# taesungp/swapping-autoencoder-pytorch

Measured on NVIDIA H100. Metric: training images/sec, higher is better.
Workload: dtype tf32

## Files before the change

### include/sae_b200.h

```cpp
#ifndef SAE_B200_H_
#define SAE_B200_H_

#include <stdint.h>

#ifdef __cplusplus
extern "C" {
#endif

#define SAE_OK              0
#define SAE_E_INVALID      -1
#define SAE_E_CUDA         -2
#define SAE_E_UNSUPPORTED  -3

#define SAE_ABI_VERSION 15
int         sae_abi_version(void);
const char* sae_last_error(void);
int64_t     sae_launch_count(void);
int         sae_tcgen05_available(void);

int sae_upfirdn2d(const float* input, const float* kernel, float* out,
                  int64_t major, int in_h, int in_w, int minor,
                  int kernel_h, int kernel_w,
                  int up_x, int up_y, int down_x, int down_y,
                  int pad_x0, int pad_x1, int pad_y0, int pad_y1,
                  int round_tf32, void* stream);

int sae_upfirdn2d_separable(const float* input, const float* taps_y, const float* taps_x, float* out,
                            int64_t major, int in_h, int in_w, int minor, int kernel_h, int kernel_w,
                            int up, int down, int pad_x0, int pad_x1, int pad_y0, int pad_y1, int round_tf32, void* stream);

int sae_fused_bias_act(const float* x, const float* bias, const float* ref, float* out,
                       int64_t size_x, int64_t step_b, int size_b,
                       int act, int grad, float alpha, float scale,
                       const float* noise, const float* noise_weight, int64_t noise_div,
                       int round_tf32, void* stream);

int sae_bias_act_backward(const float* grad_out, const float* out, float* grad_in, float* grad_bias,
// ... 45 lines not shown
} sae_conv_geom;

typedef struct sae_conv_epilogue {
    const float* bias;
    const float* noise;
    const float* noise_weight;
    const float* residual;
    float   alpha;
    float   gain;
    float   res_scale;
    int32_t act;
    int32_t round_tf32;
    uint32_t* act_mask;
} sae_conv_epilogue;

int sae_conv2d_fprop(const float* x, const float* w, float* y, const sae_conv_geom* g,
                     const sae_conv_epilogue* epi, int impl, void* stream);
int sae_conv2d_dgrad(const float* dy, const float* wt, float* dx, const sae_conv_geom* g,
                     const sae_conv_epilogue* epi, int impl, void* stream);
int sae_conv2d_wgrad(const float* dy, const float* x, float* dw, const sae_conv_geom* g,
                     int impl, void* stream);

int sae_conv2d_query_impl(const sae_conv_geom* g, int dir);

int sae_split_tf32(const float* x, float* hi, float* lo, int64_t n, void* stream);
int sae_conv2d_fprop_3xtf32(const float* x, const float* w_hi, const float* w_lo, float* y, const sae_conv_geom* g,
                            const sae_conv_epilogue* epi, int impl, void* stream);
int sae_conv2d_dgrad_3xtf32(const float* dy, const float* wt_hi, const float* wt_lo, float* dx, const sae_conv_geom* g,
                            const sae_conv_epilogue* epi, int impl, void* stream);
int sae_conv2d_wgrad_3xtf32(const float* dy, const float* x, float* dw, const sae_conv_geom* g, int impl, void* stream);

int sae_bucket_pack(const float* const* ptrs, const int64_t* offsets, const int64_t* sizes, int n,
                    float* bucket, int64_t total, void* stream);
int sae_bucket_unpack(float* const* ptrs, const int64_t* offsets, const int64_t* sizes, int n,
                      const float* bucket, int64_t total, float scale, void* stream);

int sae_filter_modulate(const float* w_krsc, const float* s, float* out_nkrsc, float* out_ncrsk, int n, int k, int c, int r,
                        int s_, int round_tf32, void* stream);
int sae_conv2d_query_modulated(const sae_conv_geom* g);
int sae_conv2d_fprop_per_sample(const float* x, const float* w_nkrsc, float* y, const sae_conv_geom* g,
                                const sae_conv_epilogue* epi, void* stream);
int sae_conv2d_dgrad_per_sample(const float* dy, const float* w_ncrsk, float* dx, const sae_conv_geom* g,
                                const sae_conv_epilogue* epi, void* stream);
int sae_conv2d_wgrad_modulated(const float* dy, const float* x, const float* s, const float* w_krsc, float* dw, float* ds,
                               const sae_conv_geom* g, void* stream);
int sae_conv2d_fprop_per_sample_3xtf32(const float* x, const float* w_nkrsc_hi, const float* w_nkrsc_lo, float* y,
// ... 61 lines not shown
```

### swapping_autoencoder_pytorch_b200/_lib.py

```python
import ctypes
import os
import subprocess
import threading

_HERE = os.path.dirname(os.path.abspath(__file__))
LIB_PATH = os.path.join(_HERE, "libsae_b200.so")
CSRC_DIR = os.path.join(_HERE, "csrc")

SAE_ABI_VERSION = 15

c_float_p = ctypes.c_void_p
c_stream = ctypes.c_void_p


class ConvGeom(ctypes.Structure):
    _fields_ = [(n, ctypes.c_int32) for n in
                ("N", "H", "W", "C", "K", "R", "S", "P", "Q", "stride", "pad_t", "pad_l")]

    def key(self):
        return tuple(getattr(self, n) for n, _ in self._fields_)


class ConvEpilogue(ctypes.Structure):
    _fields_ = [("bias", ctypes.c_void_p), ("noise", ctypes.c_void_p), ("noise_weight", ctypes.c_void_p),
                ("residual", ctypes.c_void_p), ("alpha", ctypes.c_float), ("gain", ctypes.c_float),
                ("res_scale", ctypes.c_float), ("act", ctypes.c_int32), ("round_tf32", ctypes.c_int32),
                ("act_mask", ctypes.c_void_p)]


SIGNATURES = {
    "sae_abi_version": (ctypes.c_int, []),
    "sae_last_error": (ctypes.c_char_p, []),
# ... 25 lines not shown
                                             ctypes.c_int64, ctypes.c_int, ctypes.c_int, c_stream]),
    "sae_add_scale": (ctypes.c_int, [c_float_p, c_float_p, c_float_p, ctypes.c_int64, ctypes.c_float, ctypes.c_int,
                                     c_stream]),
    "sae_round_tf32": (ctypes.c_int, [c_float_p, c_float_p, ctypes.c_int64, c_stream]),
    "sae_upsample2x_add_scale": (ctypes.c_int, [c_float_p, c_float_p, c_float_p, ctypes.c_int, ctypes.c_int, ctypes.c_int,
                                                ctypes.c_int, ctypes.c_float, ctypes.c_int, c_stream]),
    "sae_upsample2x_backward": (ctypes.c_int, [c_float_p, c_float_p, ctypes.c_int, ctypes.c_int, ctypes.c_int, ctypes.c_int,
                                               ctypes.c_float, ctypes.c_int, c_stream]),
    "sae_filter_prep": (ctypes.c_int, [c_float_p, c_float_p, c_float_p, ctypes.c_int, ctypes.c_int, ctypes.c_int, ctypes.c_int,
                                       ctypes.c_float, ctypes.c_int, c_stream]),
    "sae_filter_unprep": (ctypes.c_int, [c_float_p, c_float_p, ctypes.c_int, ctypes.c_int, ctypes.c_int, ctypes.c_int,
                                         ctypes.c_float, c_stream]),
    "sae_reflect_pad": (ctypes.c_int, [c_float_p, c_float_p] + [ctypes.c_int] * 8 + [c_stream]),
    "sae_reflect_pad_backward": (ctypes.c_int, [c_float_p, c_float_p] + [ctypes.c_int] * 8 + [c_stream]),
    "sae_pad_channels": (ctypes.c_int, [c_float_p, c_float_p, ctypes.c_int64, ctypes.c_int64, ctypes.c_int, ctypes.c_int,
                                        ctypes.c_int64, ctypes.c_int64, ctypes.c_int64, ctypes.c_int, c_stream]),
    "sae_conv2d_fprop": (ctypes.c_int, [c_float_p, c_float_p, c_float_p, ctypes.POINTER(ConvGeom),
                                        ctypes.POINTER(ConvEpilogue), ctypes.c_int, c_stream]),
    "sae_conv2d_dgrad": (ctypes.c_int, [c_float_p, c_float_p, c_float_p, ctypes.POINTER(ConvGeom),
                                        ctypes.POINTER(ConvEpilogue), ctypes.c_int, c_stream]),
    "sae_conv2d_wgrad": (ctypes.c_int, [c_float_p, c_float_p, c_float_p, ctypes.POINTER(ConvGeom), ctypes.c_int,
                                        c_stream]),
    "sae_conv2d_query_impl": (ctypes.c_int, [ctypes.POINTER(ConvGeom), ctypes.c_int]),
    "sae_split_tf32": (ctypes.c_int, [c_float_p, c_float_p, c_float_p, ctypes.c_int64, c_stream]),
    "sae_conv2d_fprop_3xtf32": (ctypes.c_int, [c_float_p, c_float_p, c_float_p, c_float_p, ctypes.POINTER(ConvGeom),
                                               ctypes.POINTER(ConvEpilogue), ctypes.c_int, c_stream]),
    "sae_conv2d_dgrad_3xtf32": (ctypes.c_int, [c_float_p, c_float_p, c_float_p, c_float_p, ctypes.POINTER(ConvGeom),
                                               ctypes.POINTER(ConvEpilogue), ctypes.c_int, c_stream]),
    "sae_conv2d_wgrad_3xtf32": (ctypes.c_int, [c_float_p, c_float_p, c_float_p, ctypes.POINTER(ConvGeom), ctypes.c_int,
                                               c_stream]),
    "sae_bucket_pack": (ctypes.c_int, [ctypes.c_void_p, ctypes.c_void_p, ctypes.c_void_p, ctypes.c_int, c_float_p,
                                       ctypes.c_int64, c_stream]),
    "sae_bucket_unpack": (ctypes.c_int, [ctypes.c_void_p, ctypes.c_void_p, ctypes.c_void_p, ctypes.c_int, c_float_p,
                                         ctypes.c_int64, ctypes.c_float, c_stream]),
    "sae_filter_modulate": (ctypes.c_int, [c_float_p] * 4 + [ctypes.c_int] * 6 + [c_stream]),
    "sae_conv2d_query_modulated": (ctypes.c_int, [ctypes.POINTER(ConvGeom)]),
    "sae_conv2d_fprop_per_sample": (ctypes.c_int, [c_float_p, c_float_p, c_float_p, ctypes.POINTER(ConvGeom),
                                                   ctypes.POINTER(ConvEpilogue), c_stream]),
    "sae_conv2d_dgrad_per_sample": (ctypes.c_int, [c_float_p, c_float_p, c_float_p, ctypes.POINTER(ConvGeom),
                                                   ctypes.POINTER(ConvEpilogue), c_stream]),
    "sae_conv2d_wgrad_modulated": (ctypes.c_int, [c_float_p] * 6 + [ctypes.POINTER(ConvGeom), c_stream]),
    "sae_conv2d_fprop_per_sample_3xtf32": (ctypes.c_int, [c_float_p, c_float_p, c_float_p, c_float_p, ctypes.POINTER(ConvGeom),
                                                          ctypes.POINTER(ConvEpilogue), c_stream]),
    "sae_conv2d_dgrad_per_sample_3xtf32": (ctypes.c_int, [c_float_p, c_float_p, c_float_p, c_float_p, ctypes.POINTER(ConvGeom),
                                                          ctypes.POINTER(ConvEpilogue), c_stream]),
    "sae_conv2d_wgrad_modulated_3xtf32": (ctypes.c_int, [c_float_p] * 6 + [ctypes.POINTER(ConvGeom), c_stream]),
# ... 68 lines not shown
```

### swapping_autoencoder_pytorch_b200/csrc/api.cu

```cuda
#include "conv_internal.cuh"
#include <mutex>

namespace sae {

thread_local char g_err[512] = "";
std::atomic<int64_t> g_launches{0};

int sm_count() {
    static int n = 0;
    static std::once_flag once;
    std::call_once(once, [] {
        int dev = 0;
        if (cudaGetDevice(&dev) != cudaSuccess) dev = 0;
        cudaDeviceProp prop;
        if (cudaGetDeviceProperties(&prop, dev) == cudaSuccess) n = prop.multiProcessorCount;
        if (n <= 0) n = 132;
    });
    return n;
}

static int validate_geom(const sae_conv_geom* g, const char* who) {
    if (!g) return fail(SAE_E_INVALID, "%s: null geometry", who);
    if (g->N < 0 || g->H <= 0 || g->W <= 0 || g->C <= 0 || g->K <= 0 || g->R <= 0 || g->S <= 0 || g->P <= 0 ||
        g->Q <= 0 || g->stride <= 0)
        return fail(SAE_E_INVALID, "%s: non-positive dimension", who);
    if ((int64_t)(g->P - 1) * g->stride - g->pad_t + g->R - 1 < 0 || (int64_t)(g->Q - 1) * g->stride - g->pad_l + g->S - 1 < 0)
        return fail(SAE_E_INVALID, "%s: inconsistent P/Q", who);
    return SAE_OK;
}

}

using namespace sae;

extern "C" int sae_abi_version(void) { return SAE_ABI_VERSION; }
extern "C" const char* sae_last_error(void) { return g_err; }
extern "C" int64_t sae_launch_count(void) { return g_launches.load(std::memory_order_relaxed); }
extern "C" int sae_tcgen05_available(void) { return tc_available() ? 1 : 0; }

extern "C" int sae_conv2d_query_impl(const sae_conv_geom* g, int dir) {
    if (validate_geom(g, "query_impl") != SAE_OK) return SAE_E_INVALID;
    if (!tc_available()) return 1;
    bool ok = dir == 0 ? tc_fprop_eligible(g) : dir == 1 ? tc_dgrad_eligible(g) : wgrad_wg_eligible(g);
    return ok ? 2 : 1;
}

static int conv2d_fprop(const float* x, const float* w, const float* w_lo, float* y, const sae_conv_geom* g,
                        const sae_conv_epilogue* epi, int impl, void* stream, const char* who,
                        void* ws = nullptr, int64_t* ws_bytes = nullptr) {
    int rc = validate_geom(g, who);
    if (rc) return rc;
    const bool det = ws_bytes != nullptr;
    bool query = false;
    if (g->N == 0) return det ? det_workspace(ws, ws_bytes, 0, who, &query) : SAE_OK;
    if (!x || !w || !y) return fail(SAE_E_INVALID, "%s: null pointer", who);
    cudaStream_t st = (cudaStream_t)stream;
    EpiParams e = make_epi(epi);
    const bool tc_ok = (det || tc_available()) && tc_fprop_eligible(g);
    if (impl == 2 && !tc_ok) return fail(SAE_E_UNSUPPORTED, "%s: shape not eligible for the wgmma kernel", who);
    if (impl != 1 && tc_ok) {
        if (det && ((rc = det_workspace(ws, ws_bytes, 0, who, &query)) || query)) return rc;
        return tc_fprop(x, w, y, g, e, st, w_lo);
    }
    GatherParams p;
    p.N = g->N; p.OH = g->P; p.OW = g->Q; p.IH = g->H; p.IW = g->W; p.Cs = g->C; p.R = g->R; p.S = g->S;
    p.SY = g->stride; p.DY = 1; p.OFFY = -g->pad_t; p.OFFX = -g->pad_l; p.DIV = 1;
    p.Ncol = g->K; p.K = g->R * g->S * g->C; p.M = (int64_t)g->N * g->P * g->Q;
// ... 204 lines not shown
```

### swapping_autoencoder_pytorch_b200/csrc/conv_internal.cuh

```cuda
#pragma once
#include "common.cuh"

namespace sae {

struct GatherParams {
    int N, OH, OW;
    int IH, IW, Cs;
    int R, S;
    int SY, DY, OFFY, OFFX, DIV;
    int Ncol;
    int K;
    int64_t M;
};

struct WgradParams {
    int N, H, W, C;
    int Ko, R, S;
    int P, Q;
    int stride, pad_t, pad_l;
    int Ncol;
    int64_t Mpix;
    int64_t chunk;
    int64_t img_pix;
    const float* mod_s;
// ... 13 lines not shown
    return row_tiles * groups_per_tile * splits_per_image * taps;
}

int conv_gather_dispatch(const float* src, const float* wmat, float* out, const GatherParams& p, const EpiParams& e,
                         cudaStream_t st, const float* wlo = nullptr);
int conv_gather_dispatch_det(const float* src, const float* wmat, float* out, const GatherParams& p, const EpiParams& e,
                             cudaStream_t st, const float* wlo, void* ws, int64_t* ws_bytes, const char* who);
int conv_wgrad(const float* dy, const float* x, float* dw, const sae_conv_geom* g, int impl, cudaStream_t st, bool split = false);
bool wgrad_modulated_eligible(const sae_conv_geom* g);
int conv_wgrad_modulated(const float* dy, const float* x, const float* s, const float* w_krsc, float* dw, float* ds,
                         const sae_conv_geom* g, cudaStream_t st, bool split = false);
int conv_wgrad_det(const float* dy, const float* x, float* dw, const sae_conv_geom* g, int impl, cudaStream_t st, bool split,
                   void* ws, int64_t* ws_bytes, const char* who);
int conv_wgrad_modulated_det(const float* dy, const float* x, const float* s, const float* w_krsc, float* dw, float* ds,
                             const sae_conv_geom* g, cudaStream_t st, bool split, void* ws, int64_t* ws_bytes, const char* who);

bool tc_available();
bool tc_fprop_eligible(const sae_conv_geom* g);
bool tc_dgrad_eligible(const sae_conv_geom* g);
int tc_fprop(const float* x, const float* w, float* y, const sae_conv_geom* g, const EpiParams& e, cudaStream_t st,
             const float* w_lo = nullptr);
int tc_dgrad(const float* dy, const float* wt, float* dx, const sae_conv_geom* g, const EpiParams& e, cudaStream_t st,
             const float* wt_lo = nullptr);
bool wgrad_wg_eligible(const sae_conv_geom* g);
int wgrad_wg_launch(const float* dy, const float* x, float* dw, const WgradParams& p, cudaStream_t st, DetWs* det = nullptr);
int wgrad_split_launch(const float* dy, const float* x, float* dw, const WgradParams& p, unsigned splits, cudaStream_t st,
                       const DetWs* det = nullptr);
bool tc_per_sample_eligible(const sae_conv_geom* g, int dgrad);
int tc_conv_per_sample(const float* src, const float* w, float* out, const sae_conv_geom* g, int dgrad, const EpiParams& e,
                       cudaStream_t st, const float* w_lo = nullptr);

}
```

### swapping_autoencoder_pytorch_b200/csrc/conv_wgmma.cu

```cuda
#include "tc_common.cuh"
#include <mutex>

namespace sae {

EncodeTiledFn g_encode = nullptr;
static bool g_tc_ok = false;

static void tc_init_once() {
    static std::once_flag once;
    std::call_once(once, [] {
        int dev = 0;
        if (cudaGetDevice(&dev) != cudaSuccess) return;
        cudaDeviceProp prop;
        if (cudaGetDeviceProperties(&prop, dev) != cudaSuccess) return;
        if (prop.major != 9) return;
        void* fn = nullptr;
        cudaDriverEntryPointQueryResult qres;
        if (cudaGetDriverEntryPoint("cuTensorMapEncodeTiled", &fn, cudaEnableDefault, &qres) != cudaSuccess) return;
        if (qres != cudaDriverEntryPointSuccess || fn == nullptr) return;
        g_encode = (EncodeTiledFn)fn;
        const char* off = getenv("SAE_DISABLE_TCGEN05");
        g_tc_ok = !(off && off[0] == '1');
    });
}
// ... 2 lines not shown
    tc_init_once();
    return g_tc_ok;
}

constexpr int TC_MAX_TAPS = 16;
constexpr int TC_THREADS = 288;
constexpr int TC_CONSUMERS = 256;
constexpr int TC_BK = 32;
constexpr int TC_A_BYTES = 128 * TC_BK * 4;

struct TcParams {
    int num_cblk;
    int ntaps;
    int stride;
    int tw, th, tn;
    int tiles_w, tiles_h, tiles_n;
    int ON, OH, OW, Ncol;
    int src_c;
    int o_mul, o_offy, o_offx;
    int FH, FW;
    short oy[TC_MAX_TAPS], ox[TC_MAX_TAPS];
    int wk[TC_MAX_TAPS];
    int w_nstride;
    EpiParams epi;
};

__device__ __forceinline__ void tc_epilogue_math(float (&v)[32], const EpiParams& e, int colb, int64_t pixel, int ncol, bool valid, float nz) {
    uint32_t pos = 0;
#pragma unroll
    for (int j = 0; j < 32; ++j) {
        float t = v[j];
        if (e.bias) t += __ldg(e.bias + colb + j);
        t += nz;
        pos |= (t > 0.f ? 1u : 0u) << j;
        if (e.act == 3) t = t > 0.f ? t : t * e.alpha;
        t *= e.gain;
        v[j] = t;
    }
    if (e.act_mask && valid) e.act_mask[(pixel * ncol + colb) >> 5] = pos;
    if (e.residual && valid) {
        const float4* r4 = reinterpret_cast<const float4*>(e.residual + pixel * ncol + colb);
#pragma unroll
        for (int j = 0; j < 8; ++j) {
            float4 r = __ldg(r4 + j);
            v[4 * j + 0] = (v[4 * j + 0] + r.x) * e.res_scale;
            v[4 * j + 1] = (v[4 * j + 1] + r.y) * e.res_scale;
// ... 173 lines not shown
        float nz = 0.f;
        if (p.epi.noise && valid) nz = __ldg(p.epi.noise_weight) * __ldg(p.epi.noise + pixel);
        uint8_t* stg = smem_gen + (size_t)ch * TC_A_BYTES + (size_t)row * 128;
        float v[32];
#pragma unroll
        for (int j = 0; j < 8; ++j) {
            const float4 o = *reinterpret_cast<const float4*>(stg + ((j ^ (row & 7)) << 4));
            v[4 * j] = o.x; v[4 * j + 1] = o.y; v[4 * j + 2] = o.z; v[4 * j + 3] = o.w;
        }
        tc_epilogue_math(v, p.epi, col0 + ch * 32, pixel, p.Ncol, valid, nz);
#pragma unroll
        for (int j = 0; j < 8; ++j)
            *reinterpret_cast<float4*>(stg + ((j ^ (row & 7)) << 4)) = make_float4(v[4 * j], v[4 * j + 1], v[4 * j + 2], v[4 * j + 3]);
    }
    asm volatile("fence.proxy.async.shared::cta;" ::: "memory");
    asm volatile("bar.sync 1, %0;" ::"n"(TC_CONSUMERS) : "memory");
    if (threadIdx.x == 0) {
        for (int ch = 0; ch < NCHUNK; ++ch) tma_store_4d(&map_out, base + (uint32_t)ch * TC_A_BYTES, col0 + ch * 32, q0, p0, n0);
        asm volatile("cp.async.bulk.commit_group;" ::: "memory");
        asm volatile("cp.async.bulk.wait_group.read 0;" ::: "memory");
    }
}

int encode_map(CUtensorMap* m, const void* ptr, int rank, const cuuint64_t* dims, const cuuint64_t* strides_bytes,
               const cuuint32_t* box, const cuuint32_t* estr, CUtensorMapSwizzle swizzle) {
    if (g_encode == nullptr && !tc_available()) return fail(SAE_E_UNSUPPORTED, "cuTensorMapEncodeTiled is not available on this device / driver");
    CUresult r = g_encode(m, CU_TENSOR_MAP_DATA_TYPE_FLOAT32, (cuuint32_t)rank, const_cast<void*>(ptr), dims, strides_bytes, box,
                          estr, CU_TENSOR_MAP_INTERLEAVE_NONE, swizzle, CU_TENSOR_MAP_L2_PROMOTION_L2_256B,
                          CU_TENSOR_MAP_FLOAT_OOB_FILL_NONE);
    if (r != CUDA_SUCCESS) return fail(SAE_E_CUDA, "cuTensorMapEncodeTiled failed with CUresult %d", (int)r);
    return SAE_OK;
}

struct TcProblem {
    const float* src; int SN, SH, SW, SC;
    const float* wmat; int Ncol, Ktot;
    const float* wmat_lo;
    int w_per_sample;
    float* out; int OH, OW;
    int o_mul, o_offy, o_offx, FH, FW;
    int stride, ntaps;
    int oy[TC_MAX_TAPS], ox[TC_MAX_TAPS], wk[TC_MAX_TAPS];
};

static bool tc_shape_ok(int src_c, int ncol, int ntaps, int stride, int ow) {
    if (src_c % 32 != 0 || ncol % 32 != 0) return false;
    if (ntaps < 1 || ntaps > TC_MAX_TAPS) return false;
    if (stride != 1 && stride != 2) return false;
    int tw = pow2_ceil(ow) < 16 ? pow2_ceil(ow) : 16;
    if (tw * stride > 256) return false;
    return true;
}

static void tc_fill_params(const TcProblem& pr, const EpiParams& e, TcParams& p) {
    p.num_cblk = pr.SC / 32;
    p.ntaps = pr.ntaps;
    p.stride = pr.stride;
    tile_box(pr.OH, pr.OW, 128, 16, p.tw, p.th, p.tn);
    p.tiles_w = (pr.OW + p.tw - 1) / p.tw;
    p.tiles_h = (pr.OH + p.th - 1) / p.th;
    p.tiles_n = (pr.SN + p.tn - 1) / p.tn;
    p.ON = pr.SN; p.OH = pr.OH; p.OW = pr.OW; p.Ncol = pr.Ncol; p.src_c = pr.SC;
    for (int t = 0; t < pr.ntaps; ++t) { p.oy[t] = (short)pr.oy[t]; p.ox[t] = (short)pr.ox[t]; p.wk[t] = pr.wk[t]; }
    p.o_mul = pr.o_mul; p.o_offy = pr.o_offy; p.o_offx = pr.o_offx; p.FH = pr.FH; p.FW = pr.FW;
    p.w_nstride = pr.w_per_sample ? pr.Ncol : 0;
    p.epi = e;
}

static int tc_encode_filter(const TcProblem& pr, const float* wmat, int b_rows, CUtensorMap* mw) {
    cuuint64_t dims[2] = {(cuuint64_t)pr.Ktot, (cuuint64_t)pr.Ncol * (cuuint64_t)(pr.w_per_sample ? pr.SN : 1)};
    cuuint64_t strides[1] = {(cuuint64_t)pr.Ktot * 4};
    cuuint32_t box[2] = {32, (cuuint32_t)b_rows};
    cuuint32_t es[2] = {1, 1};
    return encode_map(mw, wmat, 2, dims, strides, box, es);
}

int encode_act_map(CUtensorMap* m, const float* ptr, int N, int H, int W, int C, int tw, int th, int tn, int stride) {
    cuuint64_t dims[4] = {(cuuint64_t)C, (cuuint64_t)W, (cuuint64_t)H, (cuuint64_t)N};
    cuuint64_t strides[3] = {(cuuint64_t)C * 4, (cuuint64_t)W * C * 4, (cuuint64_t)H * W * C * 4};
    cuuint32_t box[4] = {32, (cuuint32_t)(tw * stride), (cuuint32_t)(th * stride), (cuuint32_t)tn};
    cuuint32_t es[4] = {1, (cuuint32_t)stride, (cuuint32_t)stride, 1};
    return encode_map(m, ptr, 4, dims, strides, box, es);
}

static int tc_encode_maps(const TcProblem& pr, const TcParams& p, int b_rows, CUtensorMap* msrc, CUtensorMap* mw, CUtensorMap* mout) {
    {
        int rc = encode_act_map(msrc, pr.src, pr.SN, pr.SH, pr.SW, pr.SC, p.tw, p.th, p.tn, pr.stride);
        if (rc) return rc;
    }
    {
        int rc = tc_encode_filter(pr, pr.wmat, b_rows, mw);
        if (rc) return rc;
    }
    {
        cuuint64_t dims[4] = {(cuuint64_t)pr.Ncol, (cuuint64_t)pr.OW, (cuuint64_t)pr.OH, (cuuint64_t)pr.SN};
        cuuint64_t strides[3] = {(cuuint64_t)pr.o_mul * pr.Ncol * 4, (cuuint64_t)pr.o_mul * pr.FW * pr.Ncol * 4,
                                 (cuuint64_t)pr.FH * pr.FW * pr.Ncol * 4};
        cuuint32_t box[4] = {32, (cuuint32_t)p.tw, (cuuint32_t)p.th, (cuuint32_t)p.tn};
        cuuint32_t es[4] = {1, 1, 1, 1};
        int rc = encode_map(mout, pr.out + ((int64_t)pr.o_offy * pr.FW + pr.o_offx) * pr.Ncol, 4, dims, strides, box, es);
        if (rc) return rc;
    }
    return SAE_OK;
}

template <int BLOCK_N, bool SPLIT>
static int tc_launch_batch(const TcProblem* prs, int count, const EpiParams& e, cudaStream_t st) {
    TcBatch b;
    if (count < 1 || count > TC_MAX_BATCH) return fail(SAE_E_INVALID, "conv_wg: batch of %d problems", count);
    b.count = count;
    int tiles = 0;
    for (int i = 0; i < count; ++i) {
        tc_fill_params(prs[i], e, b.p[i]);
        if (prs[i].w_per_sample && b.p[i].tn != 1) return fail(SAE_E_UNSUPPORTED, "conv_wg: per-sample filters need one image per tile");
        CUtensorMap mw;
        int rc = tc_encode_maps(prs[i], b.p[i], BLOCK_N, &b.src[i], &mw, &b.out[i]);
        if (rc) return rc;
        if (i == 0) b.w = mw;
        else if (prs[i].wmat != prs[0].wmat || prs[i].wmat_lo != prs[0].wmat_lo || prs[i].Ncol != prs[0].Ncol ||
                 prs[i].Ktot != prs[0].Ktot)
            return fail(SAE_E_INVALID, "conv_wg: batched problems must share the filter matrix");
        tiles += b.p[i].tiles_w * b.p[i].tiles_h * b.p[i].tiles_n;
        b.tile_end[i] = tiles;
    }
    if (SPLIT) {
        int rc = tc_encode_filter(prs[0], prs[0].wmat_lo, BLOCK_N, &b.w_lo);
        if (rc) return rc;
    }
    constexpr size_t smem = tc_smem_bytes<BLOCK_N, SPLIT>();
    static bool attr_done = false;
    if (!attr_done) {
        SAE_CUDA_TRY(cudaFuncSetAttribute(conv_wg_kernel<BLOCK_N, SPLIT>, cudaFuncAttributeMaxDynamicSharedMemorySize, (int)smem));
        attr_done = true;
    }
    dim3 grid((unsigned)tiles, (unsigned)(prs[0].Ncol / BLOCK_N));
    conv_wg_kernel<BLOCK_N, SPLIT><<<grid, TC_THREADS, smem, st>>>(b);
    return check_launch("conv_wg");
}

static int tc_dispatch(const TcProblem* prs, int count, const EpiParams& e, cudaStream_t st) {
    const int ncol = prs[0].Ncol;
    if (prs[0].wmat_lo) {
        if (ncol % 64 == 0) return tc_launch_batch<64, true>(prs, count, e, st);
        return tc_launch_batch<32, true>(prs, count, e, st);
    }
    if (ncol % 128 == 0) return tc_launch_batch<128, false>(prs, count, e, st);
    if (ncol % 64 == 0) return tc_launch_batch<64, false>(prs, count, e, st);
    return tc_launch_batch<32, false>(prs, count, e, st);
}

static bool ptr_ok(const void* a, const void* b, const void* c, const void* d = nullptr) {
    return ((reinterpret_cast<uintptr_t>(a) | reinterpret_cast<uintptr_t>(b) | reinterpret_cast<uintptr_t>(c) |
             reinterpret_cast<uintptr_t>(d)) & 15) == 0;
}

bool tc_fprop_eligible(const sae_conv_geom* g) {
    if (g->R * g->S > TC_MAX_TAPS) return false;
    if (g->pad_t > 100 || g->pad_l > 100) return false;
    return tc_shape_ok(g->C, g->K, g->R * g->S, g->stride, g->Q);
}

bool tc_dgrad_eligible(const sae_conv_geom* g) {
    if (g->stride != 1 && g->stride != 2) return false;
    if (g->R * g->S > TC_MAX_TAPS) return false;
    if (g->pad_t > 100 || g->pad_l > 100) return false;
    return tc_shape_ok(g->K, g->C, g->R * g->S, 1, (g->W + g->stride - 1) / g->stride);
}

int tc_fprop(const float* x, const float* w, float* y, const sae_conv_geom* g, const EpiParams& e, cudaStream_t st,
             const float* w_lo) {
    if (!ptr_ok(x, w, y, w_lo)) return fail(SAE_E_INVALID, "conv2d_fprop(wgmma): pointers must be 16-byte aligned");
    TcProblem pr;
    pr.w_per_sample = 0;
    pr.wmat_lo = w_lo;
    pr.src = x; pr.SN = g->N; pr.SH = g->H; pr.SW = g->W; pr.SC = g->C;
    pr.wmat = w; pr.Ncol = g->K; pr.Ktot = g->R * g->S * g->C;
    pr.out = y; pr.OH = g->P; pr.OW = g->Q;
    pr.o_mul = 1; pr.o_offy = 0; pr.o_offx = 0; pr.FH = g->P; pr.FW = g->Q;
    pr.stride = g->stride; pr.ntaps = g->R * g->S;
    for (int r = 0; r < g->R; ++r)
        for (int s = 0; s < g->S; ++s) {
            const int t = r * g->S + s;
            pr.oy[t] = r - g->pad_t; pr.ox[t] = s - g->pad_l; pr.wk[t] = t * g->C;
        }
    return tc_dispatch(&pr, 1, e, st);
}

bool tc_per_sample_eligible(const sae_conv_geom* g, int dgrad) {
    if (g->stride != 1 || g->R * g->S > TC_MAX_TAPS) return false;
    const int src_c = dgrad ? g->K : g->C, ncol = dgrad ? g->C : g->K;
    const int oh = dgrad ? g->H : g->P, ow = dgrad ? g->W : g->Q;
    if (src_c % 32 != 0 || ncol % 32 != 0 || oh % 16 != 0 || ow % 8 != 0) return false;
    if (g->R > 3 || g->S > 3) return false;
    return (int64_t)g->N * oh * ow >= 2 * 128;
}

int tc_conv_per_sample(const float* src, const float* w, float* out, const sae_conv_geom* g, int dgrad, const EpiParams& e, cudaStream_t st,
                       const float* w_lo) {
    if (!tc_per_sample_eligible(g, dgrad)) return fail(SAE_E_UNSUPPORTED, "per-sample conv: shape outside the per-sample kernel");
    if (!ptr_ok(src, w, out, w_lo)) return fail(SAE_E_INVALID, "per-sample conv: pointers must be 16-byte aligned");
    TcProblem pr;
    pr.w_per_sample = 1;
    pr.wmat_lo = w_lo;
    pr.stride = 1; pr.o_mul = 1; pr.o_offy = 0; pr.o_offx = 0; pr.ntaps = g->R * g->S;
    pr.src = src; pr.wmat = w; pr.out = out; pr.SN = g->N;
    if (!dgrad) {
        pr.SH = g->H; pr.SW = g->W; pr.SC = g->C; pr.Ncol = g->K; pr.Ktot = g->R * g->S * g->C;
        pr.OH = g->P; pr.OW = g->Q; pr.FH = g->P; pr.FW = g->Q;
    } else {
        pr.SH = g->P; pr.SW = g->Q; pr.SC = g->K; pr.Ncol = g->C; pr.Ktot = g->R * g->S * g->K;
        pr.OH = g->H; pr.OW = g->W; pr.FH = g->H; pr.FW = g->W;
    }
    for (int r = 0; r < g->R; ++r)
        for (int s_ = 0; s_ < g->S; ++s_) {
            const int t = r * g->S + s_;
            pr.oy[t] = dgrad ? g->pad_t - r : r - g->pad_t;
            pr.ox[t] = dgrad ? g->pad_l - s_ : s_ - g->pad_l;
            pr.wk[t] = t * pr.SC;
        }
    return tc_dispatch(&pr, 1, e, st);
}

__global__ void __launch_bounds__(256)
tc_dgrad_empty_kernel(float* __restrict__ dx, const EpiParams e, int64_t total, int H, int W, int C, unsigned empty) {
    for (int64_t i = blockIdx.x * (int64_t)blockDim.x + threadIdx.x; i < total; i += (int64_t)gridDim.x * blockDim.x) {
        const int64_t pixel = i / C;
        const int col = (int)(i - pixel * C);
        const int x = (int)(pixel % W), y = (int)((pixel / W) % H);
        if (!((empty >> ((y & 1) * 2 + (x & 1))) & 1u)) continue;
        float t = 0.f;
        if (e.bias) t += __ldg(e.bias + col);
        if (e.noise) t += __ldg(e.noise_weight) * __ldg(e.noise + pixel);
        const uint32_t pos = __ballot_sync(0xffffffffu, t > 0.f);
        if (e.act == 3) t = t > 0.f ? t : t * e.alpha;
        t *= e.gain;
        if (e.act_mask && (i & 31) == 0) e.act_mask[i >> 5] = pos;
        if (e.residual) t = (t + __ldg(e.residual + i)) * e.res_scale;
        if (e.round_tf32) t = rna_tf32(t);
        dx[i] = t;
    }
}

int tc_dgrad(const float* dy, const float* wt, float* dx, const sae_conv_geom* g, const EpiParams& e, cudaStream_t st,
             const float* wt_lo) {
    if (!ptr_ok(dy, wt, dx, wt_lo)) return fail(SAE_E_INVALID, "conv2d_dgrad(wgmma): pointers must be 16-byte aligned");
    TcProblem pr;
    pr.w_per_sample = 0;
    pr.wmat_lo = wt_lo;
    pr.src = dy; pr.SN = g->N; pr.SH = g->P; pr.SW = g->Q; pr.SC = g->K;
    pr.wmat = wt; pr.Ncol = g->C; pr.Ktot = g->R * g->S * g->K;
    pr.stride = 1; pr.FH = g->H; pr.FW = g->W;
    const int st_ = g->stride;
    if (st_ == 1) {
        pr.out = dx; pr.OH = g->H; pr.OW = g->W; pr.o_mul = 1; pr.o_offy = 0; pr.o_offx = 0;
        pr.ntaps = g->R * g->S;
        for (int r = 0; r < g->R; ++r)
            for (int s = 0; s < g->S; ++s) {
                const int t = r * g->S + s;
                pr.oy[t] = g->pad_t - r; pr.ox[t] = g->pad_l - s; pr.wk[t] = t * g->K;
            }
        return tc_dispatch(&pr, 1, e, st);
    }
    unsigned empty = 0;
    for (int ho = 0; ho < 2; ++ho)
        for (int wo = 0; wo < 2; ++wo) {
            const int rp = (ho + g->pad_t) & 1, sp = (wo + g->pad_l) & 1;
            if (rp >= g->R || sp >= g->S) empty |= 1u << (ho * 2 + wo);
        }
    if (empty) {
        const int64_t total = (int64_t)g->N * g->H * g->W * g->C;
        if (!e.bias && !e.noise && !e.residual && !e.act_mask) {
            SAE_CUDA_TRY(cudaMemsetAsync(dx, 0, (size_t)total * sizeof(float), st));
        } else {
            int64_t blocks = (total + 255) / 256;
            if (blocks > (int64_t)sm_count() * 16) blocks = (int64_t)sm_count() * 16;
            tc_dgrad_empty_kernel<<<(unsigned)blocks, 256, 0, st>>>(dx, e, total, g->H, g->W, g->C, empty);
            int rc = check_launch("conv_wg(dgrad, empty parity classes)");
            if (rc) return rc;
        }
    }
    TcProblem cls_pr[TC_MAX_BATCH];
    int ncls = 0;
    for (int ho = 0; ho < 2; ++ho)
        for (int wo = 0; wo < 2; ++wo) {
            const int rp = (ho + g->pad_t) & 1, sp = (wo + g->pad_l) & 1;
            if (rp >= g->R || sp >= g->S) continue;
            if (ho >= g->H || wo >= g->W) continue;
            pr.out = dx; pr.o_mul = 2; pr.o_offy = ho; pr.o_offx = wo;
            pr.OH = (g->H - ho + 1) / 2; pr.OW = (g->W - wo + 1) / 2;
            int nt = 0;
            for (int r = rp; r < g->R; r += 2)
                for (int s = sp; s < g->S; s += 2) {
                    const int ny = ho + g->pad_t - r, nx = wo + g->pad_l - s;
                    pr.oy[nt] = ny >= 0 ? ny / 2 : -((-ny) / 2);
                    pr.ox[nt] = nx >= 0 ? nx / 2 : -((-nx) / 2);
                    pr.wk[nt] = (r * g->S + s) * g->K;
                    ++nt;
                }
            pr.ntaps = nt;
            cls_pr[ncls++] = pr;
        }
    if (ncls == 0) return SAE_OK;
    return tc_dispatch(cls_pr, ncls, e, st);
}

}
```

Measured before the change: 137.7.

## Add 256-row wide-tile WGMMA conv kernel with two consumer warpgroups

Adds a warp-specialized conv kernel that computes 256-row by 128-column output tiles, using two consumer warpgroups that share each TMA-loaded filter tile and a 4-stage ring. A heuristic picks it over the 128-row kernel when Ncol is a multiple of 128, K is deep enough, there are enough tiles to fill the SMs, and the padding waste stays small. The goal is better filter reuse and fewer tiles per FLOP on large convolutions. The cost is fewer resident blocks and a larger shared-memory footprint. The change also adds a query API that reports which tile size is chosen.

New measurement: 152.8 (median of 6 runs). 1.11x the previous value.

```diff
diff --git a/include/sae_b200.h b/include/sae_b200.h
--- a/include/sae_b200.h
+++ b/include/sae_b200.h
@@ -12,7 +12,7 @@
 #define SAE_E_CUDA         -2
 #define SAE_E_UNSUPPORTED  -3
 
-#define SAE_ABI_VERSION 15
+#define SAE_ABI_VERSION 16
 int         sae_abi_version(void);
 const char* sae_last_error(void);
 int64_t     sae_launch_count(void);
@@ -104,6 +104,7 @@
                      int impl, void* stream);
 
 int sae_conv2d_query_impl(const sae_conv_geom* g, int dir);
+int sae_conv2d_query_tile(const sae_conv_geom* g, int dir, int per_sample);
 
 int sae_split_tf32(const float* x, float* hi, float* lo, int64_t n, void* stream);
 int sae_conv2d_fprop_3xtf32(const float* x, const float* w_hi, const float* w_lo, float* y, const sae_conv_geom* g,
diff --git a/swapping_autoencoder_pytorch_b200/_lib.py b/swapping_autoencoder_pytorch_b200/_lib.py
--- a/swapping_autoencoder_pytorch_b200/_lib.py
+++ b/swapping_autoencoder_pytorch_b200/_lib.py
@@ -7,7 +7,7 @@
 LIB_PATH = os.path.join(_HERE, "libsae_b200.so")
 CSRC_DIR = os.path.join(_HERE, "csrc")
 
-SAE_ABI_VERSION = 15
+SAE_ABI_VERSION = 16
 
 c_float_p = ctypes.c_void_p
 c_stream = ctypes.c_void_p
@@ -79,6 +79,7 @@
     "sae_conv2d_wgrad": (ctypes.c_int, [c_float_p, c_float_p, c_float_p, ctypes.POINTER(ConvGeom), ctypes.c_int,
                                         c_stream]),
     "sae_conv2d_query_impl": (ctypes.c_int, [ctypes.POINTER(ConvGeom), ctypes.c_int]),
+    "sae_conv2d_query_tile": (ctypes.c_int, [ctypes.POINTER(ConvGeom), ctypes.c_int, ctypes.c_int]),
     "sae_split_tf32": (ctypes.c_int, [c_float_p, c_float_p, c_float_p, ctypes.c_int64, c_stream]),
     "sae_conv2d_fprop_3xtf32": (ctypes.c_int, [c_float_p, c_float_p, c_float_p, c_float_p, ctypes.POINTER(ConvGeom),
                                                ctypes.POINTER(ConvEpilogue), ctypes.c_int, c_stream]),
diff --git a/swapping_autoencoder_pytorch_b200/csrc/api.cu b/swapping_autoencoder_pytorch_b200/csrc/api.cu
--- a/swapping_autoencoder_pytorch_b200/csrc/api.cu
+++ b/swapping_autoencoder_pytorch_b200/csrc/api.cu
@@ -43,6 +43,13 @@
     if (!tc_available()) return 1;
     bool ok = dir == 0 ? tc_fprop_eligible(g) : dir == 1 ? tc_dgrad_eligible(g) : wgrad_wg_eligible(g);
     return ok ? 2 : 1;
+}
+
+extern "C" int sae_conv2d_query_tile(const sae_conv_geom* g, int dir, int per_sample) {
+    if (validate_geom(g, "query_tile") != SAE_OK) return SAE_E_INVALID;
+    if (dir != 0 && dir != 1) return fail(SAE_E_INVALID, "query_tile: dir must be 0 (fprop) or 1 (dgrad)");
+    if (!tc_available()) return 0;
+    return tc_query_tile(g, dir, per_sample);
 }
 
 static int conv2d_fprop(const float* x, const float* w, const float* w_lo, float* y, const sae_conv_geom* g,
diff --git a/swapping_autoencoder_pytorch_b200/csrc/conv_internal.cuh b/swapping_autoencoder_pytorch_b200/csrc/conv_internal.cuh
--- a/swapping_autoencoder_pytorch_b200/csrc/conv_internal.cuh
+++ b/swapping_autoencoder_pytorch_b200/csrc/conv_internal.cuh
@@ -59,6 +59,7 @@
              const float* w_lo = nullptr);
 int tc_dgrad(const float* dy, const float* wt, float* dx, const sae_conv_geom* g, const EpiParams& e, cudaStream_t st,
              const float* wt_lo = nullptr);
+int tc_query_tile(const sae_conv_geom* g, int dir, int per_sample);
 bool wgrad_wg_eligible(const sae_conv_geom* g);
 int wgrad_wg_launch(const float* dy, const float* x, float* dw, const WgradParams& p, cudaStream_t st, DetWs* det = nullptr);
 int wgrad_split_launch(const float* dy, const float* x, float* dw, const WgradParams& p, unsigned splits, cudaStream_t st,
diff --git a/swapping_autoencoder_pytorch_b200/csrc/conv_wgmma.cu b/swapping_autoencoder_pytorch_b200/csrc/conv_wgmma.cu
--- a/swapping_autoencoder_pytorch_b200/csrc/conv_wgmma.cu
+++ b/swapping_autoencoder_pytorch_b200/csrc/conv_wgmma.cu
@@ -48,6 +48,8 @@
     short oy[TC_MAX_TAPS], ox[TC_MAX_TAPS];
     int wk[TC_MAX_TAPS];
     int w_nstride;
+    int oth, otn;
+    int odh, odn;
     EpiParams epi;
 };
 
@@ -267,6 +269,149 @@
     }
 }
 
+constexpr int WIDE_STAGES = 4;
+constexpr int WIDE_A_BYTES = 256 * TC_BK * 4;
+constexpr int WIDE_B_BYTES = 128 * TC_BK * 4;
+constexpr int WIDE_STAGE_BYTES = WIDE_A_BYTES + WIDE_B_BYTES;
+constexpr uint32_t WIDE_RING = (uint32_t)WIDE_STAGES * WIDE_STAGE_BYTES;
+constexpr uint32_t WIDE_EPI = 2u * TC_A_BYTES;
+constexpr size_t WIDE_SMEM = (size_t)WIDE_RING + WIDE_EPI + 1024  + 256 ;
+constexpr int WIDE_THREADS = 384;
+
+__global__ void __launch_bounds__(WIDE_THREADS, 1)
+conv_wide_kernel(const __grid_constant__ TcBatch batch, const int ncb) {
+    extern __shared__ uint8_t smem_raw[];
+    const uint32_t base = (smem_u32(smem_raw) + 1023u) & ~1023u;
+    const uint32_t bar_full = base + WIDE_RING + WIDE_EPI;
+    const uint32_t bar_empty = bar_full + 8 * WIDE_STAGES;
+    uint8_t* smem_gen = smem_raw + (base - smem_u32(smem_raw));
+    const int warp = threadIdx.x >> 5, lane = threadIdx.x & 31;
+    const int total = batch.tile_end[batch.count - 1] * ncb;
+
+    if (threadIdx.x == 0) {
+        for (int s = 0; s < WIDE_STAGES; ++s) {
+            mbar_init(bar_full + 8 * s, 1);
+            mbar_init(bar_empty + 8 * s, TC_CONSUMERS / 32);
+        }
+        asm volatile("fence.mbarrier_init.release.cluster;" ::: "memory");
+    }
+    __syncthreads();
+
+    auto decode = [&](int t, int& prob, int& q0, int& p0, int& n0, int& col0) {
+        int pt = t / ncb;
+        col0 = (t - pt * ncb) * 128;
+        prob = 0;
+        while (prob + 1 < batch.count && pt >= batch.tile_end[prob]) ++prob;
+        if (prob > 0) pt -= batch.tile_end[prob - 1];
+        const TcParams& p = batch.p[prob];
+        q0 = (pt % p.tiles_w) * p.tw; pt /= p.tiles_w;
+        p0 = (pt % p.tiles_h) * p.th;
+        n0 = (pt / p.tiles_h) * p.tn;
+    };
+
+    if (warp >= TC_CONSUMERS / 32) {
+        asm volatile("setmaxnreg.dec.sync.aligned.u32 40;" ::: "memory");
+        if (warp == TC_CONSUMERS / 32 && lane == 0) {
+            uint32_t it = 0;
+            for (int t = blockIdx.x; t < total; t += gridDim.x) {
+                int prob, q0, p0, n0, col0;
+                decode(t, prob, q0, p0, n0, col0);
+                const TcParams& p = batch.p[prob];
+                const int wrow = col0 + n0 * p.w_nstride;
+                const int KB = p.ntaps * p.num_cblk;
+                for (int kb = 0; kb < KB; ++kb, ++it) {
+                    const uint32_t s = it % WIDE_STAGES;
+                    mbar_wait(bar_empty + 8 * s, ((it / WIDE_STAGES) & 1u) ^ 1u);
+                    const int tap = kb / p.num_cblk, cb = kb - tap * p.num_cblk;
+                    const uint32_t sa = base + s * WIDE_STAGE_BYTES, sb = sa + WIDE_A_BYTES;
+                    mbar_expect_tx(bar_full + 8 * s, WIDE_STAGE_BYTES);
+                    tma_load_4d(sa, &batch.src[prob], bar_full + 8 * s, cb * TC_BK, q0 * p.stride + p.ox[tap],
+                                p0 * p.stride + p.oy[tap], n0);
+                    tma_load_2d(sb, &batch.w, bar_full + 8 * s, p.wk[tap] + cb * TC_BK, wrow);
+                }
+            }
+        }
+        return;
+    }
+
+    asm volatile("setmaxnreg.inc.sync.aligned.u32 232;" ::: "memory");
+    const int wg = warp >> 2, wtid = threadIdx.x & 127;
+    const uint32_t stg = base + WIDE_RING + (uint32_t)wg * TC_A_BYTES;
+    uint8_t* const stg_gen = smem_gen + WIDE_RING + (size_t)wg * TC_A_BYTES;
+    uint32_t it = 0;
+    for (int t = blockIdx.x; t < total; t += gridDim.x) {
+        int prob, q0, p0, n0, col0;
+        decode(t, prob, q0, p0, n0, col0);
+        const TcParams& p = batch.p[prob];
+        const int KB = p.ntaps * p.num_cblk;
+        float acc[2][64];
+#pragma unroll
+        for (int i = 0; i < 64; ++i) { acc[0][i] = 0.f; acc[1][i] = 0.f; }
+        for (int kb = 0; kb < KB; ++kb, ++it) {
+            const uint32_t s = it % WIDE_STAGES;
+            mbar_wait(bar_full + 8 * s, (it / WIDE_STAGES) & 1u);
+            const uint32_t sa = base + s * WIDE_STAGE_BYTES + (uint32_t)wg * (128 * 128);
+            const uint64_t da0 = make_wgmma_desc_sw128(sa), da1 = make_wgmma_desc_sw128(sa + 64 * 128);
+            const uint64_t db = make_wgmma_desc_sw128(base + s * WIDE_STAGE_BYTES + WIDE_A_BYTES);
+            wgmma_fence();
+#pragma unroll
+            for (int k = 0; k < TC_BK / 8; ++k) {
+                wgmma_tf32_n128(acc[0], da0 + (uint64_t)(k * 2), db + (uint64_t)(k * 2));
+                wgmma_tf32_n128(acc[1], da1 + (uint64_t)(k * 2), db + (uint64_t)(k * 2));
+            }
+            wgmma_commit();
+            wgmma_wait<1>();
+            if (kb > 0 && lane == 0) mbar_arrive(bar_empty + 8 * ((it - 1) % WIDE_STAGES));
+        }
+        wgmma_wait<0>();
+        if (lane == 0) mbar_arrive(bar_empty + 8 * ((it - 1) % WIDE_STAGES));
+
+        const int R = wg * 128 + wtid;
+        const int iw = R % p.tw, ih = (R / p.tw) % p.th, in_ = R / (p.tw * p.th);
+        const int n = n0 + in_, pp = p0 + ih, qq = q0 + iw;
+        const bool valid = n < p.ON && pp < p.OH && qq < p.OW;
+        const int64_t pixel = ((int64_t)n * p.FH + pp * p.o_mul + p.o_offy) * p.FW + qq * p.o_mul + p.o_offx;
+        float nz = 0.f;
+        if (p.epi.noise && valid) nz = __ldg(p.epi.noise_weight) * __ldg(p.epi.noise + pixel);
+#pragma unroll
+        for (int ch = 0; ch < 4; ++ch) {
+            if (wtid == 0) asm volatile("cp.async.bulk.wait_group.read 0;" ::: "memory");
+            asm volatile("bar.sync %0, 128;" ::"r"(1 + wg) : "memory");
+#pragma unroll
+            for (int m = 0; m < 2; ++m)
+#pragma unroll
+                for (int jj = 0; jj < 4; ++jj) {
+                    const int j = 4 * ch + jj, col = 8 * jj + 2 * (lane & 3), piece = col >> 2;
+#pragma unroll
+                    for (int h = 0; h < 2; ++h) {
+                        const int row = 64 * m + (warp & 3) * 16 + (lane >> 2) + 8 * h;
+                        uint8_t* dst = stg_gen + (size_t)row * 128 + ((piece ^ (row & 7)) << 4) + (col & 3) * 4;
+                        *reinterpret_cast<float2*>(dst) = make_float2(acc[m][4 * j + 2 * h], acc[m][4 * j + 2 * h + 1]);
+                    }
+                }
+            asm volatile("bar.sync %0, 128;" ::"r"(1 + wg) : "memory");
+            uint8_t* const srow = stg_gen + (size_t)wtid * 128;
+            float v[32];
+#pragma unroll
+            for (int j = 0; j < 8; ++j) {
+                const float4 o = *reinterpret_cast<const float4*>(srow + ((j ^ (wtid & 7)) << 4));
+                v[4 * j] = o.x; v[4 * j + 1] = o.y; v[4 * j + 2] = o.z; v[4 * j + 3] = o.w;
+            }
+            tc_epilogue_math(v, p.epi, col0 + ch * 32, pixel, p.Ncol, valid, nz);
+#pragma unroll
+            for (int j = 0; j < 8; ++j)
+                *reinterpret_cast<float4*>(srow + ((j ^ (wtid & 7)) << 4)) = make_float4(v[4 * j], v[4 * j + 1], v[4 * j + 2], v[4 * j + 3]);
+            asm volatile("fence.proxy.async.shared::cta;" ::: "memory");
+            asm volatile("bar.sync %0, 128;" ::"r"(1 + wg) : "memory");
+            if (wtid == 0) {
+                tma_store_4d(&batch.out[prob], stg, col0 + ch * 32, q0, p0 + wg * p.odh, n0 + wg * p.odn);
+                asm volatile("cp.async.bulk.commit_group;" ::: "memory");
+            }
+        }
+    }
+    if (wtid == 0) asm volatile("cp.async.bulk.wait_group.read 0;" ::: "memory");
+}
+
 int encode_map(CUtensorMap* m, const void* ptr, int rank, const cuuint64_t* dims, const cuuint64_t* strides_bytes,
                const cuuint32_t* box, const cuuint32_t* estr, CUtensorMapSwizzle swizzle) {
     if (g_encode == nullptr && !tc_available()) return fail(SAE_E_UNSUPPORTED, "cuTensorMapEncodeTiled is not available on this device / driver");
@@ -297,11 +442,16 @@
     return true;
 }
 
-static void tc_fill_params(const TcProblem& pr, const EpiParams& e, TcParams& p) {
+static void tc_fill_params(const TcProblem& pr, const EpiParams& e, TcParams& p, int rows) {
     p.num_cblk = pr.SC / 32;
     p.ntaps = pr.ntaps;
     p.stride = pr.stride;
-    tile_box(pr.OH, pr.OW, 128, 16, p.tw, p.th, p.tn);
+    tile_box(pr.OH, pr.OW, rows, 16, p.tw, p.th, p.tn);
+    p.oth = p.th; p.otn = p.tn; p.odh = 0; p.odn = 0;
+    if (rows == 256) {
+        if (p.tn >= 2) p.otn = p.odn = p.tn / 2;
+        else p.oth = p.odh = p.th / 2;
+    }
     p.tiles_w = (pr.OW + p.tw - 1) / p.tw;
     p.tiles_h = (pr.OH + p.th - 1) / p.th;
     p.tiles_n = (pr.SN + p.tn - 1) / p.tn;
@@ -341,7 +491,7 @@
         cuuint64_t dims[4] = {(cuuint64_t)pr.Ncol, (cuuint64_t)pr.OW, (cuuint64_t)pr.OH, (cuuint64_t)pr.SN};
         cuuint64_t strides[3] = {(cuuint64_t)pr.o_mul * pr.Ncol * 4, (cuuint64_t)pr.o_mul * pr.FW * pr.Ncol * 4,
                                  (cuuint64_t)pr.FH * pr.FW * pr.Ncol * 4};
-        cuuint32_t box[4] = {32, (cuuint32_t)p.tw, (cuuint32_t)p.th, (cuuint32_t)p.tn};
+        cuuint32_t box[4] = {32, (cuuint32_t)p.tw, (cuuint32_t)p.oth, (cuuint32_t)p.otn};
         cuuint32_t es[4] = {1, 1, 1, 1};
         int rc = encode_map(mout, pr.out + ((int64_t)pr.o_offy * pr.FW + pr.o_offx) * pr.Ncol, 4, dims, strides, box, es);
         if (rc) return rc;
@@ -356,7 +506,7 @@
     b.count = count;
     int tiles = 0;
     for (int i = 0; i < count; ++i) {
-        tc_fill_params(prs[i], e, b.p[i]);
+        tc_fill_params(prs[i], e, b.p[i], 128);
         if (prs[i].w_per_sample && b.p[i].tn != 1) return fail(SAE_E_UNSUPPORTED, "conv_wg: per-sample filters need one image per tile");
         CUtensorMap mw;
         int rc = tc_encode_maps(prs[i], b.p[i], BLOCK_N, &b.src[i], &mw, &b.out[i]);
@@ -383,8 +533,58 @@
     return check_launch("conv_wg");
 }
 
+constexpr int WIDE_MIN_TILES = DET_SMS;
+static int tc_tile_rows(const TcProblem* prs, int count) {
+    if (prs[0].wmat_lo || prs[0].Ncol % 128 != 0) return 128;
+    if (prs[0].Ktot < (prs[0].Ncol == 128 ? 32 : 4) * TC_BK) return 128;
+    int64_t tiles = 0, wide_rows = 0, narrow_rows = 0;
+    for (int i = 0; i < count; ++i) {
+        const TcProblem& pr = prs[i];
+        int tw, th, tn;
+        tile_box(pr.OH, pr.OW, 256, 16, tw, th, tn);
+        if (th * pr.stride > 256) return 128;
+        if (pr.w_per_sample && tn != 1) return 128;
+        const int64_t wide = (int64_t)((pr.OW + tw - 1) / tw) * ((pr.OH + th - 1) / th) * ((pr.SN + tn - 1) / tn);
+        tile_box(pr.OH, pr.OW, 128, 16, tw, th, tn);
+        tiles += wide;
+        wide_rows += 256 * wide;
+        narrow_rows += 128 * (int64_t)((pr.OW + tw - 1) / tw) * ((pr.OH + th - 1) / th) * ((pr.SN + tn - 1) / tn);
+    }
+    if (tiles * (prs[0].Ncol / 128) < WIDE_MIN_TILES || 16 * wide_rows > 17 * narrow_rows) return 128;
+    return 256;
+}
+
+static int tc_launch_wide(const TcProblem* prs, int count, const EpiParams& e, cudaStream_t st) {
+    TcBatch b;
+    if (count < 1 || count > TC_MAX_BATCH) return fail(SAE_E_INVALID, "conv_wide: batch of %d problems", count);
+    b.count = count;
+    int tiles = 0;
+    for (int i = 0; i < count; ++i) {
+        tc_fill_params(prs[i], e, b.p[i], 256);
+        CUtensorMap mw;
+        int rc = tc_encode_maps(prs[i], b.p[i], 128, &b.src[i], &mw, &b.out[i]);
+        if (rc) return rc;
+        if (i == 0) b.w = mw;
+        else if (prs[i].wmat != prs[0].wmat || prs[i].Ncol != prs[0].Ncol || prs[i].Ktot != prs[0].Ktot)
+            return fail(SAE_E_INVALID, "conv_wide: batched problems must share the filter matrix");
+        tiles += b.p[i].tiles_w * b.p[i].tiles_h * b.p[i].tiles_n;
+        b.tile_end[i] = tiles;
+    }
+    static bool attr_done = false;
+    if (!attr_done) {
+        SAE_CUDA_TRY(cudaFuncSetAttribute(conv_wide_kernel, cudaFuncAttributeMaxDynamicSharedMemorySize, (int)WIDE_SMEM));
+        attr_done = true;
+    }
+    const int ncb = prs[0].Ncol / 128;
+    const int64_t total = (int64_t)tiles * ncb;
+    const int grid = total < sm_count() ? (int)total : sm_count();
+    conv_wide_kernel<<<grid, WIDE_THREADS, WIDE_SMEM, st>>>(b, ncb);
+    return check_launch("conv_wide");
+}
+
 static int tc_dispatch(const TcProblem* prs, int count, const EpiParams& e, cudaStream_t st) {
     const int ncol = prs[0].Ncol;
+    if (tc_tile_rows(prs, count) == 256) return tc_launch_wide(prs, count, e, st);
     if (prs[0].wmat_lo) {
         if (ncol % 64 == 0) return tc_launch_batch<64, true>(prs, count, e, st);
         return tc_launch_batch<32, true>(prs, count, e, st);
@@ -412,10 +612,7 @@
     return tc_shape_ok(g->K, g->C, g->R * g->S, 1, (g->W + g->stride - 1) / g->stride);
 }
 
-int tc_fprop(const float* x, const float* w, float* y, const sae_conv_geom* g, const EpiParams& e, cudaStream_t st,
-             const float* w_lo) {
-    if (!ptr_ok(x, w, y, w_lo)) return fail(SAE_E_INVALID, "conv2d_fprop(wgmma): pointers must be 16-byte aligned");
-    TcProblem pr;
+static void fprop_problem(const float* x, const float* w, const float* w_lo, float* y, const sae_conv_geom* g, TcProblem& pr) {
     pr.w_per_sample = 0;
     pr.wmat_lo = w_lo;
     pr.src = x; pr.SN = g->N; pr.SH = g->H; pr.SW = g->W; pr.SC = g->C;
@@ -428,6 +625,13 @@
             const int t = r * g->S + s;
             pr.oy[t] = r - g->pad_t; pr.ox[t] = s - g->pad_l; pr.wk[t] = t * g->C;
         }
+}
+
+int tc_fprop(const float* x, const float* w, float* y, const sae_conv_geom* g, const EpiParams& e, cudaStream_t st,
+             const float* w_lo) {
+    if (!ptr_ok(x, w, y, w_lo)) return fail(SAE_E_INVALID, "conv2d_fprop(wgmma): pointers must be 16-byte aligned");
+    TcProblem pr;
+    fprop_problem(x, w, w_lo, y, g, pr);
     return tc_dispatch(&pr, 1, e, st);
 }
 
@@ -440,11 +644,8 @@
     return (int64_t)g->N * oh * ow >= 2 * 128;
 }
 
-int tc_conv_per_sample(const float* src, const float* w, float* out, const sae_conv_geom* g, int dgrad, const EpiParams& e, cudaStream_t st,
-                       const float* w_lo) {
-    if (!tc_per_sample_eligible(g, dgrad)) return fail(SAE_E_UNSUPPORTED, "per-sample conv: shape outside the per-sample kernel");
-    if (!ptr_ok(src, w, out, w_lo)) return fail(SAE_E_INVALID, "per-sample conv: pointers must be 16-byte aligned");
-    TcProblem pr;
+static void per_sample_problem(const float* src, const float* w, const float* w_lo, float* out, const sae_conv_geom* g, int dgrad,
+                               TcProblem& pr) {
     pr.w_per_sample = 1;
     pr.wmat_lo = w_lo;
     pr.stride = 1; pr.o_mul = 1; pr.o_offy = 0; pr.o_offx = 0; pr.ntaps = g->R * g->S;
@@ -463,6 +664,14 @@
             pr.ox[t] = dgrad ? g->pad_l - s_ : s_ - g->pad_l;
             pr.wk[t] = t * pr.SC;
         }
+}
+
+int tc_conv_per_sample(const float* src, const float* w, float* out, const sae_conv_geom* g, int dgrad, const EpiParams& e, cudaStream_t st,
+                       const float* w_lo) {
+    if (!tc_per_sample_eligible(g, dgrad)) return fail(SAE_E_UNSUPPORTED, "per-sample conv: shape outside the per-sample kernel");
+    if (!ptr_ok(src, w, out, w_lo)) return fail(SAE_E_INVALID, "per-sample conv: pointers must be 16-byte aligned");
+    TcProblem pr;
+    per_sample_problem(src, w, w_lo, out, g, dgrad, pr);
     return tc_dispatch(&pr, 1, e, st);
 }
 
@@ -486,17 +695,16 @@
     }
 }
 
-int tc_dgrad(const float* dy, const float* wt, float* dx, const sae_conv_geom* g, const EpiParams& e, cudaStream_t st,
-             const float* wt_lo) {
-    if (!ptr_ok(dy, wt, dx, wt_lo)) return fail(SAE_E_INVALID, "conv2d_dgrad(wgmma): pointers must be 16-byte aligned");
+static int dgrad_problems(const float* dy, const float* wt, const float* wt_lo, float* dx, const sae_conv_geom* g,
+                          TcProblem (&cls_pr)[TC_MAX_BATCH], unsigned& empty) {
     TcProblem pr;
     pr.w_per_sample = 0;
     pr.wmat_lo = wt_lo;
     pr.src = dy; pr.SN = g->N; pr.SH = g->P; pr.SW = g->Q; pr.SC = g->K;
     pr.wmat = wt; pr.Ncol = g->C; pr.Ktot = g->R * g->S * g->K;
     pr.stride = 1; pr.FH = g->H; pr.FW = g->W;
-    const int st_ = g->stride;
-    if (st_ == 1) {
+    empty = 0;
+    if (g->stride == 1) {
         pr.out = dx; pr.OH = g->H; pr.OW = g->W; pr.o_mul = 1; pr.o_offy = 0; pr.o_offx = 0;
         pr.ntaps = g->R * g->S;
         for (int r = 0; r < g->R; ++r)
@@ -504,27 +712,14 @@
                 const int t = r * g->S + s;
                 pr.oy[t] = g->pad_t - r; pr.ox[t] = g->pad_l - s; pr.wk[t] = t * g->K;
             }
-        return tc_dispatch(&pr, 1, e, st);
-    }
-    unsigned empty = 0;
+        cls_pr[0] = pr;
+        return 1;
+    }
     for (int ho = 0; ho < 2; ++ho)
         for (int wo = 0; wo < 2; ++wo) {
             const int rp = (ho + g->pad_t) & 1, sp = (wo + g->pad_l) & 1;
             if (rp >= g->R || sp >= g->S) empty |= 1u << (ho * 2 + wo);
         }
-    if (empty) {
-        const int64_t total = (int64_t)g->N * g->H * g->W * g->C;
-        if (!e.bias && !e.noise && !e.residual && !e.act_mask) {
-            SAE_CUDA_TRY(cudaMemsetAsync(dx, 0, (size_t)total * sizeof(float), st));
-        } else {
-            int64_t blocks = (total + 255) / 256;
-            if (blocks > (int64_t)sm_count() * 16) blocks = (int64_t)sm_count() * 16;
-            tc_dgrad_empty_kernel<<<(unsigned)blocks, 256, 0, st>>>(dx, e, total, g->H, g->W, g->C, empty);
-            int rc = check_launch("conv_wg(dgrad, empty parity classes)");
-            if (rc) return rc;
-        }
-    }
-    TcProblem cls_pr[TC_MAX_BATCH];
     int ncls = 0;
     for (int ho = 0; ho < 2; ++ho)
         for (int wo = 0; wo < 2; ++wo) {
@@ -545,8 +740,47 @@
             pr.ntaps = nt;
             cls_pr[ncls++] = pr;
         }
+    return ncls;
+}
+
+int tc_dgrad(const float* dy, const float* wt, float* dx, const sae_conv_geom* g, const EpiParams& e, cudaStream_t st,
+             const float* wt_lo) {
+    if (!ptr_ok(dy, wt, dx, wt_lo)) return fail(SAE_E_INVALID, "conv2d_dgrad(wgmma): pointers must be 16-byte aligned");
+    TcProblem cls_pr[TC_MAX_BATCH];
+    unsigned empty;
+    const int ncls = dgrad_problems(dy, wt, wt_lo, dx, g, cls_pr, empty);
+    if (empty) {
+        const int64_t total = (int64_t)g->N * g->H * g->W * g->C;
+        if (!e.bias && !e.noise && !e.residual && !e.act_mask) {
+            SAE_CUDA_TRY(cudaMemsetAsync(dx, 0, (size_t)total * sizeof(float), st));
+        } else {
+            int64_t blocks = (total + 255) / 256;
+            if (blocks > (int64_t)sm_count() * 16) blocks = (int64_t)sm_count() * 16;
+            tc_dgrad_empty_kernel<<<(unsigned)blocks, 256, 0, st>>>(dx, e, total, g->H, g->W, g->C, empty);
+            int rc = check_launch("conv_wg(dgrad, empty parity classes)");
+            if (rc) return rc;
+        }
+    }
     if (ncls == 0) return SAE_OK;
     return tc_dispatch(cls_pr, ncls, e, st);
 }
 
-}
+int tc_query_tile(const sae_conv_geom* g, int dir, int per_sample) {
+    TcProblem prs[TC_MAX_BATCH];
+    int count = 1;
+    if (per_sample) {
+        if (!tc_per_sample_eligible(g, dir)) return 0;
+        per_sample_problem(nullptr, nullptr, nullptr, nullptr, g, dir, prs[0]);
+    } else if (dir == 0) {
+        if (!tc_fprop_eligible(g)) return 0;
+        fprop_problem(nullptr, nullptr, nullptr, nullptr, g, prs[0]);
+    } else {
+        if (!tc_dgrad_eligible(g)) return 0;
+        unsigned empty;
+        count = dgrad_problems(nullptr, nullptr, nullptr, nullptr, g, prs, empty);
+        if (count == 0) return 0;
+    }
+    return tc_tile_rows(prs, count);
+}
+
+}
```
